# fanzyflani/pwnfps

Hardware: AMD Instinct MI355X
Metric: Mpixels/s at 3840x2160 (level.txt scene, trace + blur), frames resident on the device; mean steps/ray alongside; d2h_inclusive = the rate with every frame delivered to the host (SURVEY 8d) (higher is better)
Workload: dtype f32; 1 GPU; pwnfps level.txt scene (14 game.lua spheres, spawn pose, sec_current=0), 3840x2160, POSTPROC_BLUR=1, one frame per step; level=pwnfps_level, width=3840, height=2160, blur_passes=1, parallelism=rows/1, 3 frames in flight on two compute streams, frames_repeated_with_whole_strips=0

## Files before the change

pwnfps_amd/csrc/level_host.c:

```c
#include <stdint.h>
#include <stdlib.h>
#include <string.h>
#include "level_host.h"

enum { DIR_XP = 0, DIR_ZP, DIR_XN, DIR_ZN };

static int is_open(int c)
{
	switch(c)
	{
		case ';': case '$': case '"': case '#': case '&':
		case '>': case '<': case '^': case ',':
			return 1;
	}
	return 0;
}

static int flat_cell(const uint8_t *cells, int x, int z)
{
	int i = z * 64 + x;
	return (i >= 0 && i < 4096) ? cells[i] : '.';
}

static const int dir_dx[4] = { 1, 0, -1, 0 };
static const int dir_dz[4] = { 0, 1, 0, -1 };

static int open_dir(const uint8_t *cells, int x, int z)
{
	for(int d = 0; d < 4; d++)
		if(is_open(flat_cell(cells, x + dir_dx[d], z + dir_dz[d])))
			return d;
	return DIR_XP;
}

static void endpoint(pwn_portal *pm, int x, int z)
{
	if(pm->x1 == -1) { pm->x1 = x; pm->z1 = z; }
	else if(pm->x2 == -1) { pm->x2 = x; pm->z2 = z; }
}

void pwn_level_clear(uint8_t *cells, pwn_portal *pmap, int32_t *spawn)
{
	memset(cells, '.', 4096);
	for(int i = 0; i < 26; i++)
	{
		pmap[i].x1 = pmap[i].z1 = pmap[i].x2 = pmap[i].z2 = -1;
		pmap[i].rot12 = 0;
		pmap[i].c1 = pmap[i].c2 = ';';
	}
	spawn[0] = spawn[1] = 0;
}

int pwn_parse_level(const char *text, int len, uint8_t *cells, pwn_portal *pmap, int32_t *spawn)
{
	if(text == NULL || len < 0) return -1;
	pwn_level_clear(cells, pmap, spawn);

	const unsigned char *p = (const unsigned char *)text, *end = p + len;
	int x = 0, z = 0;
	while(p < end && z < 64)
	{
		int c = *p++;
		if(c == '\r' || c == '\n')
		{
			if(x != 0) { x = 0; z++; }
			continue;
		}
		if(c == '*') { spawn[0] = x; spawn[1] = z; c = ';'; }
		if(c >= 'a' && c < 'z')
		{
			endpoint(&pmap[c - 'a'], x, z);
			c = c - 'a' + 'A' + 1;
		}
		if(c >= 'A' && c <= 'Z') endpoint(&pmap[c - 'A'], x, z);
		cells[z * 64 + x] = (uint8_t)c;
		if(++x == 64) { x = 0; z++; }
	}

	for(int i = 0; i < 26; i++)
	{
		pwn_portal *pm = &pmap[i];
		if(pm->x2 == -1) continue;
		int d1 = open_dir(cells, pm->x1, pm->z1);
		int d2 = open_dir(cells, pm->x2, pm->z2);
		pm->rot12 = (d2 - d1 + 2) & 3;
		pm->c1 = flat_cell(cells, pm->x1 + dir_dx[d1], pm->z1 + dir_dz[d1]);
		pm->c2 = flat_cell(cells, pm->x2 + dir_dx[d2], pm->z2 + dir_dz[d2]);
	}
	return 0;
}

static int trunc_to_int(float f)
{
	return (f >= -2147483648.0f && f < 2147483648.0f) ? (int)f : INT32_MIN;
}

int pwn_bin_spheres(const pwn_sphere *s, int n, int32_t *off, int32_t *idx, int idx_cap)
{
	int32_t *fill = calloc(4096, sizeof(int32_t));
	if(fill == NULL) return -2;
	memset(off, 0, 4097 * sizeof(int32_t));
	for(int pass = 0; pass < 2; pass++)
	{
		for(int i = 0; i < n; i++)
		{
			int x1 = trunc_to_int(s[i].x - s[i].r), z1 = trunc_to_int(s[i].z - s[i].r);
			int x2 = trunc_to_int(s[i].x + s[i].r), z2 = trunc_to_int(s[i].z + s[i].r);
			if(x1 < 0) x1 = 0;
			if(z1 < 0) z1 = 0;
			if(x2 > 63) x2 = 63;
			if(z2 > 63) z2 = 63;
			for(int z = z1; z <= z2; z++)
			for(int x = x1; x <= x2; x++)
			{
				int c = z * 64 + x;
				if(pass == 0) off[c + 1]++;
				else idx[off[c] + fill[c]++] = i;
			}
		}
		if(pass == 0)
		{
			for(int c = 0; c < 4096; c++) off[c + 1] += off[c];
			if(idx == NULL) { free(fill); return off[4096]; }
			if(off[4096] > idx_cap) { free(fill); return -1; }
		}
	}
	free(fill);
	return off[4096];
}
```

pwnfps_amd/csrc/level_host.h:

```cpp
#ifndef PWN_LEVEL_HOST_H
#define PWN_LEVEL_HOST_H
#include <stdint.h>
#include "pwnhip.h"
#ifdef __cplusplus
extern "C" {
#endif
void pwn_level_clear(uint8_t *cells, pwn_portal *pmap, int32_t *spawn);
int pwn_parse_level(const char *text, int len, uint8_t *cells, pwn_portal *pmap, int32_t *spawn);
int pwn_bin_spheres(const pwn_sphere *s, int n, int32_t *off, int32_t *idx, int idx_cap);
#ifdef __cplusplus
}
#endif
#endif
```

pwnfps_amd/csrc/pwn_api.cpp:

```cpp
#include <hip/hip_runtime.h>
#include <stdint.h>
#include <stdio.h>
#include <stdlib.h>
#include <string.h>
#include <time.h>
#include <new>
#include <vector>
#include <xmmintrin.h>

#include "pwnhip.h"
#include "pwn_internal.h"
#include "level_host.h"
#include "approx_tables.inc"

extern "C" const char *pwn_strerror(int code)
{
	switch(code)
	{
		case PWN_OK: return "ok";
		case PWN_EINVAL: return "invalid argument";
		case PWN_ENODEV: return "no usable HIP device";
		case PWN_ENOMEM: return "out of memory";
		case PWN_EIO: return "level file could not be read";
		case PWN_EHIP: return "HIP runtime error";
// ... 241 lines not shown

extern "C" int pwn_set_option(pwn_ctx *c, int option, int value)
{
	if(GRP_HEAD(c)) return pwn_group_set_option(c, option, value);
	if(c == NULL) return PWN_EINVAL;
	switch(option)
	{
		case PWN_OPT_BLUR_PASSES:
			if(value < 0 || value > 16) return PWN_EINVAL;
			if(c->tiled != NULL) return PWN_EBUSY;
			for(int i = 0; i < c->nslots; i++) if(c->slot[i].in_flight) return PWN_EBUSY;
			c->blur_passes = value; return PWN_OK;
		case PWN_OPT_COUNTERS: c->counters_on = value ? 1 : 0; return PWN_OK;
		case PWN_OPT_SCHEDULER:
			if(value < 0 || value > PWN_SCHED_REFILL) return PWN_EINVAL;
			if(value != c->scheduler) c->blob_dirty = true;
			c->scheduler = value; return PWN_OK;
		case PWN_OPT_WAVE_LOG: c->wave_log_on = value ? 1 : 0; return PWN_OK;
		case PWN_OPT_FRAME_TIMING: if(value < 0) return PWN_EINVAL; c->frame_timing = value; return PWN_OK;
		case PWN_OPT_REFILL_LIMIT: if(value < 1 || value > 64000) return PWN_EINVAL; c->refill_limit = value; return PWN_OK;
		case PWN_OPT_UNIT_ORDER: if(value != 0 && value != 1) return PWN_EINVAL; c->unit_order = value; for(int i = 0; i < 4; i++) c->order[i].perm_valid = false; return PWN_OK;
		case PWN_OPT_TILED_CHOREO:
			if(value != PWN_TILED_CHOREO_INSTREAM && value != PWN_TILED_CHOREO_SPLIT) return PWN_EINVAL;
			if(c->tiled != NULL) return PWN_EBUSY;
			c->tiled_choreo = value; return PWN_OK;
		case PWN_OPT_TILED_COMMS:
			if(value != PWN_TILED_COMMS_ONE && value != PWN_TILED_COMMS_PER_STREAM) return PWN_EINVAL;
			if(c->tiled != NULL) return PWN_EBUSY;
			c->tiled_comms = value; return PWN_OK;
		case PWN_OPT_TILED_STREAMS:
			if(value != 2 && value != 3) return PWN_EINVAL;
			if(c->tiled != NULL) return PWN_EBUSY;
			c->tiled_streams = value; return PWN_OK;
		case PWN_OPT_TRACE_ROOM: if(value < -1 || value > 4096) return PWN_EINVAL; memset(&c->room, 0, sizeof(c->room)); c->room.mode = value; return PWN_OK;
		case PWN_OPT_CALL_STRIPS:
			if(value < -1 || value == 1 || value > PWN_CALL_STRIPS_MAX) return PWN_EINVAL;
			c->call_strips = value; c->strip_backoff = 0; c->strip_reach = 0; return PWN_OK;
		case PWN_OPT_FRAME_OVERLAP:
			for(int i = 0; i < c->nslots; i++) if(c->slot[i].in_flight) return PWN_EBUSY;
			c->frame_overlap = value ? 1 : 0; return PWN_OK;
	}
	return PWN_EINVAL;
}


static void expand_tables(uint16_t *rcp, uint16_t *rsq)
{
	for(int i = 0; i < 2048; i++)
	{
		rcp[i] = (uint16_t)(pwn_host_rcp_tab[i] ^ 0x1000u);
		rsq[i] = (uint16_t)(pwn_host_rsqrt_tab[i ^ 0x400] ^ 0x1000u);
	}
}

static int pack_blob(pwn_ctx *c)
{
	uint32_t nsph = (uint32_t)c->spheres.size();
	uint32_t nbin = 0;
	for(int i = 0; i < 4096; i++)
	{
		uint32_t cnt = (uint32_t)(c->bin_off[i + 1] - c->bin_off[i]);
		if(cnt) nbin += cnt + 1u;
	}
	if(nbin > 32767u || nsph * 32u >= PWN_LIST_END) return PWN_ETOOBIG;
	uint32_t total = (pwn_t_total(nbin, nsph) + 15u) & ~15u;
	if(total > PWN_BLOB_MAX) return PWN_ETOOBIG;
	uint32_t nrec = (uint32_t)c->bin_off[4096];
	bool inl = false;
	{
		const uint32_t total_inl = (pwn_t_total_inl(nrec, nsph) + 15u) & ~15u;
		const uint32_t extra = pwn_trace_lds_extra();
		const uint32_t fit_idx = 155648u / ((total + extra + 2047u) & ~2047u), fit_inl = 155648u / ((total_inl + extra + 2047u) & ~2047u);
		inl = c->scheduler == PWN_SCHED_UNITS && nrec > 0u && total_inl <= PWN_BLOB_MAX && fit_inl >= (fit_idx < 5u ? fit_idx : 5u);
		if(c->dbg_sphere_lists == 1) inl = false;
		if(c->dbg_sphere_lists == 2) inl = c->scheduler == PWN_SCHED_UNITS && nrec > 0u && total_inl <= PWN_BLOB_MAX;
		if(inl) total = total_inl;
	}
	c->blob.assign(total, 0);
	uint8_t *b = c->blob.data();
	uint32_t *ci = (uint32_t *)(b + PWN_T_CELLINFO);
	uint16_t *bi = (uint16_t *)(b + PWN_T_BINIDX);
	if(!c->cell_base_ok)
	{
		uint32_t *cb = c->cell_base;
		memset(cb, 0, sizeof(c->cell_base));
		for(int z = 0; z < 64; z++)
		for(int x = 0; x < 64; x++)
			cb[z * PWN_GRID_PITCH + x] = (uint32_t)c->cells[z * 64 + x] | pwn_cell_class(c->cells[z * 64 + x]);
		for(int z = 0; z < 64; z++) cb[z * PWN_GRID_PITCH + 64] = cb[z * PWN_GRID_PITCH];
		for(int x = 0; x <= 64; x++) cb[64 * PWN_GRID_PITCH + x] = cb[x];
		c->cell_base_ok = true;
	}
	memcpy(ci, c->cell_base, sizeof(c->cell_base));
	uint32_t at = 0;
	for(int i = 0; i < 4096 && !inl; i++)
	{
		int32_t k0 = c->bin_off[i], k1 = c->bin_off[i + 1];
		if(k1 > k0)
		{
			ci[(i >> 6) * PWN_GRID_PITCH + (i & 63)] |= PWN_C_SPH | (at << 16);
			for(int32_t k = k0; k < k1; k++) bi[at++] = (uint16_t)(c->bin_idx[k] * 32);
			bi[at++] = (uint16_t)PWN_LIST_END;
		}
	}
	if(inl)
	{
		float *rec = (float *)(b + PWN_T_BINIDX);
		uint16_t *which = (uint16_t *)(b + pwn_t_recsph_offset(nrec));
		for(int i = 0; i < 4096; i++)
		{
			const int32_t k0 = c->bin_off[i], k1 = c->bin_off[i + 1];
			if(k1 <= k0) continue;
			ci[(i >> 6) * PWN_GRID_PITCH + (i & 63)] |= PWN_C_SPH | ((uint32_t)k0 << 16);
			for(int32_t k = k0; k < k1; k++)
			{
				const pwn_sphere &q = c->spheres[(size_t)c->bin_idx[k]];
				float r2 = q.r * q.r;
				if(r2 < 1.17549435e-38f) r2 = 0.0f;
				rec[4 * k + 0] = q.x; rec[4 * k + 1] = q.y; rec[4 * k + 2] = q.z;
				uint32_t wbits;
				memcpy(&wbits, &r2, 4);
				if(k == k1 - 1) wbits |= 0x80000000u;
				memcpy(&rec[4 * k + 3], &wbits, 4);
				which[k] = (uint16_t)(c->bin_idx[k] * 32);
			}
		}
	}
	memcpy(b + PWN_T_RCP, c->tabs, 4096);
	memcpy(b + PWN_T_RSQ, c->tabs + 2048, 4096);
	pwn_fill_faces((float *)(b + PWN_T_FACES));
	uint32_t *pm = (uint32_t *)(b + PWN_T_PMAP);
	for(int i = 0; i < 26; i++)
	{
		const pwn_portal &p = c->pmap[i];
		pm[2 * i] = (uint32_t)(p.x1 & 0xff) | ((uint32_t)(p.z1 & 0xff) << 8) | ((uint32_t)(p.x2 & 0xff) << 16) | ((uint32_t)(p.z2 & 0xff) << 24);
		pm[2 * i + 1] = (uint32_t)(p.rot12 & 0xff) | ((uint32_t)(p.c1 & 0xff) << 8) | ((uint32_t)(p.c2 & 0xff) << 16);
	}
	c->off_sph = inl ? pwn_t_sph_offset_inl(nrec) : pwn_t_sph_offset(nbin);
	c->off_recsph = inl ? pwn_t_recsph_offset(nrec) : 0u;
	{
		float *sp = (float *)(b + c->off_sph);
		for(uint32_t i = 0; i < nsph; i++, sp += 8)
		{
			const pwn_sphere &q = c->spheres[i];
			float r2 = q.r * q.r;
			if(r2 < 1.17549435e-38f) r2 = 0.0f;
			sp[0] = q.x; sp[1] = q.y; sp[2] = q.z; sp[3] = r2;
			sp[4] = q.refl; sp[5] = q.cb; sp[6] = q.cg; sp[7] = q.cr;
		}
	}

	const int nb = (c->blob_cur + 1) % PWN_NBLOB;
	const uint32_t from = c->blob_has_static[nb] ? PWN_T_CELLINFO : 0u;
	const unsigned st = c->stage_next++ % PWN_NSTAGE;
	if(c->stage_used[st]) HIPCHK(c, hipEventSynchronize(c->ev_stage[st]));
	memcpy(c->h_stage[st], b + from, total - from);
	if(c->tables_in_use[nb]) HIPCHK(c, hipStreamWaitEvent(c->up_stream, c->tables_wait[nb], 0));
	HIPCHK(c, pwn_launch_upload(c->h_stage[st], c->d_blob[nb] + from, total - from, c->up_stream));
	HIPCHK(c, hipEventRecord(c->ev_stage[st], c->up_stream));
	HIPCHK(c, hipEventRecord(c->ev_upload[nb], c->up_stream));
	c->stage_used[st] = true;
	c->upload_pending[nb] = true;
	c->blob_has_static[nb] = true;
	c->blob_cur = nb;
	c->blob_dirty = false;
	return PWN_OK;
}

static int valid_portals(const pwn_portal *pm)
{
	for(int i = 0; i < 26; i++)
	{
		const int32_t v[4] = { pm[i].x1, pm[i].z1, pm[i].x2, pm[i].z2 };
		for(int k = 0; k < 4; k++) if(v[k] < -1 || v[k] > 63) return 0;
	}
	return 1;
}

extern "C" int pwn_upload_level(pwn_ctx *c, const uint8_t data[4096], const pwn_portal pmap[26])
{
	if(GRP_HEAD(c)) return (data == NULL || pmap == NULL) ? PWN_EINVAL : pwn_group_upload_level(c, data, pmap);
	if(c == NULL || data == NULL || pmap == NULL || !valid_portals(pmap)) return PWN_EINVAL;
	(void)hipSetDevice(c->device);
	memcpy(c->cells, data, 4096);
	memcpy(c->pmap, pmap, sizeof(c->pmap));
	c->have_level = true;
	c->cell_base_ok = false;
	c->blob_dirty = true;
	return pack_blob(c);
}

extern "C" int pwn_level_load_mem(pwn_ctx *c, const char *text, int len)
{
	if(GRP_HEAD(c)) return (text == NULL || len < 0) ? PWN_EINVAL : pwn_group_level_mem(c, text, len);
	if(c == NULL || text == NULL || len < 0) return PWN_EINVAL;
	(void)hipSetDevice(c->device);
	if(pwn_parse_level(text, len, c->cells, c->pmap, c->spawn) != 0) return PWN_EINVAL;
	c->have_level = true;
	c->cell_base_ok = false;
	c->blob_dirty = true;
	return pack_blob(c);
}

extern "C" int pwn_level_load(pwn_ctx *c, const char *path)
{
	if(c == NULL || path == NULL) return PWN_EINVAL;
	FILE *fp = fopen(path, "rb");
	if(fp == NULL) { snprintf(c->err, sizeof(c->err), "cannot open %s", path); return PWN_EIO; }
	std::vector<char> buf(1 << 20);
	size_t n = fread(buf.data(), 1, buf.size(), fp);
	fclose(fp);
	return pwn_level_load_mem(c, buf.data(), (int)n);
}

extern "C" int pwn_get_level(pwn_ctx *c, uint8_t data[4096], pwn_portal pmap[26], int32_t spawn[2])
{
	if(GRP_HEAD(c)) return pwn_get_level(GRP_M0(c), data, pmap, spawn);
	if(c == NULL) return PWN_EINVAL;
	if(data) memcpy(data, c->cells, 4096);
	if(pmap) memcpy(pmap, c->pmap, sizeof(c->pmap));
	if(spawn) { spawn[0] = c->spawn[0]; spawn[1] = c->spawn[1]; }
	return PWN_OK;
}

enum { OBJ_INVAL = 0, OBJ_FREE = 1, OBJ_SPHERE = 2 };

static int upload_live(pwn_ctx *c, const pwn_sphere *s, int n);

extern "C" int pwn_upload_spheres(pwn_ctx *c, const pwn_sphere *s, int n)
{
	if(GRP_HEAD(c)) return (n < 0 || n > PWN_OBJ_MAX || (n > 0 && s == NULL)) ? PWN_EINVAL : pwn_group_upload_spheres(c, s, n);
	if(c == NULL || n < 0 || n > PWN_OBJ_MAX || (n > 0 && s == NULL)) return PWN_EINVAL;
	int rc = upload_live(c, s, n);
	if(rc == PWN_OK)
	{
		c->objs.assign(s, s + n);
		c->obj_typ.assign((size_t)n, OBJ_SPHERE);
	}
	return rc;
}

extern "C" int pwn_obj_new(pwn_ctx *c)
{
	if(GRP_HEAD(c)) { const int r = pwn_obj_new(GRP_M0(c)); if(r < 0) snprintf(c->err, sizeof(c->err), "%s", GRP_M0(c)->err); return r; }
	if(c == NULL) return PWN_EINVAL;
	for(size_t i = 0; i < c->obj_typ.size(); i++)
		if(c->obj_typ[i] == OBJ_FREE) { c->obj_typ[i] = OBJ_INVAL; return (int)i; }
	if(c->obj_typ.size() >= (size_t)PWN_OBJ_MAX)
	{
		snprintf(c->err, sizeof(c->err), "obj_new: all %d object slots are taken", PWN_OBJ_MAX);
		return PWN_ENOMEM;
	}
	c->objs.push_back(pwn_sphere());
	c->obj_typ.push_back(OBJ_INVAL);
	return (int)c->obj_typ.size() - 1;
}

static bool obj_ok(pwn_ctx *c, int obj, const char *who)
{
	if(c == NULL) return false;
	if(obj >= 0 && (size_t)obj < c->obj_typ.size()) return true;
	snprintf(c->err, sizeof(c->err), "%s: %d is not an object", who, obj);
	return false;
}

// ... 1230 lines not shown
```

pwnfps_amd/csrc/pwn_internal.h:

```cpp
#pragma once
#include <hip/hip_runtime.h>
#include <stdint.h>
#include <stdio.h>
#include <vector>
#include <atomic>

#include "pwnhip.h"
#include "tables.h"

struct pwn_views_launch
{
	const pwn_view_rec *d_recs;
	int n;
	bool has_w;
	unsigned long long plane;
};

struct pwn_rays_launch
{
	const float *d_rays;
	const uint32_t *d_seeds;
	uint32_t n;
	bool has_w;
};
// ... 20 lines not shown
	int views;
};

extern "C" hipError_t pwn_launch_trace(const pwn_trace_params *P, int grid, size_t lds_bytes, bool count, hipStream_t stream);
extern "C" hipError_t pwn_launch_trace_refill(const pwn_trace_params *P, int grid, size_t lds_bytes, bool count, hipStream_t stream);
extern "C" unsigned pwn_trace_refill_lds_extra(bool has_w);
extern "C" int pwn_trace_refill_blocks_per_cu(size_t lds_bytes, bool count, bool has_w);
extern "C" int pwn_trace_blocks_per_cu(size_t lds_bytes, bool count, bool has_w);
extern "C" int pwn_trace_tile_h(void);
extern "C" int pwn_trace_tile_w(void);
extern "C" unsigned pwn_trace_lds_extra(void);
extern "C" hipError_t pwn_launch_blur(const pwn_blur_params *P, hipStream_t stream);
extern "C" hipError_t pwn_launch_order(const uint16_t *cost, uint32_t units, uint32_t cap, uint32_t *perm, hipStream_t stream);
extern "C" hipError_t pwn_launch_upscale(const uint32_t *src, uint32_t *dst, int w, int h, int scale, int pitch, hipStream_t stream);
extern "C" hipError_t pwn_launch_upload(const void *h_pinned_src, void *d_dst, size_t bytes, hipStream_t stream);
extern "C" hipError_t pwn_launch_words(const uint32_t *d_all, const uint32_t *d_own, uint32_t *h_pinned_dst, int world, hipStream_t stream);
extern "C" hipError_t pwn_launch_probe(int op, const uint32_t *in, uint32_t *out, int n, const uint16_t *tabs, hipStream_t stream);

#define PWN_BLOB_MAX (72u * 1024u)
#ifndef PWN_NBLOB
#define PWN_NBLOB 4
#endif
#define PWN_NCOUNTERS 48
#define PWN_TILED_STREAMS_DEFAULT 2
#define PWN_TICKET_SETS 6u
#define PWN_NSTAGE 4
#define PWN_CALL_STRIPS_MAX 32
#define PWN_HOST_REGS_MAX 16

struct pwn_slot
{
	uint32_t *d_out; float *d_z; uint32_t *d_surface;
	uint32_t *h_sbuf; float *h_zbuf; uint32_t *h_surface;
	hipEvent_t ev_k[4];
	hipEvent_t ev_done;
	bool in_flight, timed, beside;
	float sec;
	uint64_t seq;
};

struct pwn_room_ctl
{
	int mode;
	int arm, best;
	int skip, hold;
	double sum[2]; int cnt[2];
	double t_prev, t_hold;
	unsigned long long looks, switches;
};
int pwn_room_for_launch(struct pwn_ctx *c);
void pwn_room_frame_done(struct pwn_ctx *c);

struct pwn_tiled;
struct pwn_group;

#define PWN_HUB_RING 64
struct pwn_hub_post { void *dst; size_t bytes; hipEvent_t ev_free; int device; };
struct pwn_hub_box
{
	std::atomic<unsigned long long> posted, copied, consumed;
	pwn_hub_post post[PWN_HUB_RING];
	hipEvent_t done[PWN_HUB_RING];
};
struct pwn_hub
{
	int world;
	std::atomic<int> failed;
	std::atomic<unsigned> bar_count, bar_gen;
	struct pwn_ctx *member[PWN_TILED_MAX_WORLD];
	pwn_hub_box *boxes;
};
int pwn_hub_meet(pwn_hub *h, int wait_ms);

struct pwn_ctx
{
	int device, w, h;
	int num_cus;
	int blur_passes, counters_on, scheduler, refill_limit;
	bool have_level;

	uint8_t cells[4096];
	uint32_t cell_base[65 * 65];
	bool cell_base_ok;
	pwn_portal pmap[26];
	int32_t spawn[2];
	std::vector<pwn_sphere> spheres;
	std::vector<int32_t> bin_off, bin_idx;
	std::vector<pwn_sphere> objs;
	std::vector<uint8_t> obj_typ;

	std::vector<uint8_t> blob;
	uint8_t *d_blob[PWN_NBLOB]; int blob_cur;
	bool blob_has_static[PWN_NBLOB];
	hipEvent_t ev_tables[PWN_NBLOB]; bool tables_in_use[PWN_NBLOB];
	hipEvent_t tables_wait[PWN_NBLOB];
	hipEvent_t ev_upload[PWN_NBLOB]; bool upload_pending[PWN_NBLOB];
	uint8_t *h_stage[PWN_NSTAGE]; hipEvent_t ev_stage[PWN_NSTAGE]; bool stage_used[PWN_NSTAGE]; unsigned stage_next;
	hipStream_t up_stream;
	uint16_t tabs[4096];
	uint32_t off_sph;
	uint32_t off_recsph; int dbg_sphere_lists;
	bool blob_dirty;
	size_t occ_lds[8]; int occ_blocks[8];

	uint32_t *d_pre, *d_out;
	float *d_z;
	uint2 *d_skip;
	unsigned long long *d_counters;
	unsigned long long *d_wave_log; int wave_log_on; size_t wave_log_cap;
	struct unit_order_state
	{
		hipStream_t key; bool used; unsigned long long stamp;
		uint16_t *d_cost; uint32_t *d_perm; size_t cost_cap, perm_cap;
		uint32_t units, qcap; int y0, y1;
		bool cost_fresh;
		uint32_t perm_units; int perm_y0, perm_y1; bool perm_valid;
	} order[4];
	unsigned long long order_stamp;
	int tiled_choreo;
	int tiled_streams;
	int tiled_comms;
	int unit_order;
	unsigned long long order_used, order_sorts;
	bool dbg_force_hasw; int dbg_blocks_per_cu;
	int dbg_blur_th, dbg_blur_tw, dbg_blur_batch;
	int grid_reserve;
	uint32_t *d_vpre, *d_vout; float *d_vz; int views_cap;
	pwn_view_rec *h_vrec, *d_vrec; int vrec_cap;
	unsigned char *h_rays, *d_rays; size_t rays_cap;
	uint32_t *d_tickets; unsigned ticket_set;
	uint32_t *d_scratch; size_t scratch_cap;

	hipStream_t stream;
	hipStream_t stream2;
	uint32_t *d_pre2;
	pwn_room_ctl room;
	int frame_overlap;
	hipEvent_t last_frame_done; hipStream_t last_frame_stream;
	hipStream_t copy_stream;
	hipEvent_t ev[4];
	int call_strips;
	hipStream_t copy_stream2;
	int strip_copy_streams;
	int strip_calib_n; double strip_calib_ms[16];
	hipEvent_t strip_ev[2 * PWN_CALL_STRIPS_MAX]; int strip_ev_n;
	uint32_t *d_strip_miss, *h_strip_miss;
	int strips_last;
	int strip_reach;
	int strip_backoff;
	unsigned long long strip_calls, strip_redone;
	struct host_reg { void *base; size_t bytes; } host_regs[PWN_HOST_REGS_MAX]; int host_regs_n;
	pwn_stats stats;

	int nslots, frame_flags, frame_scale, frame_pitch, frame_timing;
	pwn_slot slot[PWN_MAX_SLOTS];
	uint64_t frame_seq;

	pwn_group *grp; bool grp_head;
	pwn_hub *hub;
	pwn_tiled *tiled;
	int tiled_init_ms, tiled_wait_ms;

	hipStream_t launch_stream[3]; hipEvent_t launch_event[3];
	unsigned long long launch_waits;
	int launch_rot;

// ... 42 lines not shown
```

pwnfps_amd/csrc/tables.h:

```cpp
#pragma once
#include <stdint.h>

#define PWN_GRID_PITCH 65u
#define PWN_T_RCP      0u
#define PWN_T_RSQ      4096u
#define PWN_T_FACES    8192u
#define PWN_T_EXP2     8448u
#define PWN_T_CELLINFO 8704u
#define PWN_T_PMAP     25616u
#define PWN_T_BINIDX   25824u

#define PWN_RCP_BASE   0x7e800000u
#define PWN_RSQ_BASE   0x5f000000u

#define PWN_C_ROOM   0x0100u
#define PWN_C_ROOM2  0x0200u
#define PWN_C_FOG    0x0400u
#define PWN_C_DQ     0x0800u
#define PWN_C_RAMP   0x1000u
#define PWN_C_RAMPX  0x2000u
#define PWN_C_RAMPM  0x4000u
#define PWN_C_PORTAL 0x8000u
#define PWN_C_SPH    0x80000000u
#define PWN_LIST_END 0xffffu

static inline uint32_t pwn_t_sph_offset(uint32_t nbin)
{
	return PWN_T_BINIDX + ((nbin * 2u + 15u) & ~15u);
}
static inline uint32_t pwn_t_total(uint32_t nbin, uint32_t nsph)
{
	return pwn_t_sph_offset(nbin) + nsph * 32u;
}
static inline uint32_t pwn_t_recsph_offset(uint32_t nrec) { return PWN_T_BINIDX + nrec * 16u; }
static inline uint32_t pwn_t_sph_offset_inl(uint32_t nrec) { return pwn_t_recsph_offset(nrec) + ((nrec * 2u + 15u) & ~15u); }
static inline uint32_t pwn_t_total_inl(uint32_t nrec, uint32_t nsph) { return pwn_t_sph_offset_inl(nrec) + nsph * 32u; }

#define PWN_EXP2F_TAB_INIT { \
	0x3ff0000000000000, 0x3fefd9b0d3158574, 0x3fefb5586cf9890f, 0x3fef9301d0125b51, \
	0x3fef72b83c7d517b, 0x3fef54873168b9aa, 0x3fef387a6e756238, 0x3fef1e9df51fdee1, \
	0x3fef06fe0a31b715, 0x3feef1a7373aa9cb, 0x3feedea64c123422, 0x3feece086061892d, \
	0x3feebfdad5362a27, 0x3feeb42b569d4f82, 0x3feeab07dd485429, 0x3feea47eb03a5585, \
	0x3feea09e667f3bcd, 0x3fee9f75e8ec5f74, 0x3feea11473eb0187, 0x3feea589994cce13, \
	0x3feeace5422aa0db, 0x3feeb737b0cdc5e5, 0x3feec49182a3f090, 0x3feed503b23e255d, \
	0x3feee89f995ad3ad, 0x3feeff76f2fb5e47, 0x3fef199bdd85529c, 0x3fef3720dcef9069, \
	0x3fef5818dcfba487, 0x3fef7c97337b9b5f, 0x3fefa4afa2a490da, 0x3fefd0765b6e4540 }

static inline void pwn_fill_faces(float *f)
{
	static const float col[4][4] = { { 30.0f, 30.0f, 0.0f, 0.0f }, { 1.0f, 1.0f, 1.0f, 0.0f }, { 0.8f, 0.8f, 1.0f, 0.0f }, { 5.0f, 0.0f, 5.0f, 0.0f } };
	for(int i = 0; i < 16; i++) f[i] = col[i >> 2][i & 3];
	uint32_t *u = (uint32_t *)(f + 16);
	const uint32_t S = 0x80000000u, P = 0x3a83126fu , N = 0xba83126fu, Z = 0x80000000u ;
	const uint32_t R25 = 0x3e800000u , R70 = 0x3f333333u ;
	const uint32_t t[6][8] = {
		{ S, 0, 0, R25,  N, Z, Z, 0 },
		{ 0, 0, S, R25,  Z, Z, N, 0 },
		{ S, 0, 0, R25,  P, Z, Z, S },
		{ 0, 0, S, R25,  Z, Z, P, S },
		{ 0, S, 0, R25,  Z, N, Z, 0 },
		{ 0, 0, 0, R70,  Z, N, Z, S },
	};
	for(int i = 0; i < 48; i++) u[i] = t[i >> 3][i & 7];
	static const uint64_t e2[32] = PWN_EXP2F_TAB_INIT;
	uint64_t *e = (uint64_t *)(f + (PWN_T_EXP2 - PWN_T_FACES) / 4u);
	for(int i = 0; i < 32; i++) e[i] = e2[i];
}

static inline uint32_t pwn_cell_class(uint32_t c)
{
	switch(c)
	{
		case ';': return PWN_C_ROOM;
		case '$': return PWN_C_ROOM | PWN_C_FOG;
		case '"': return PWN_C_ROOM | PWN_C_DQ;
		case '#': return PWN_C_ROOM | PWN_C_ROOM2;
		case '&': return PWN_C_ROOM | PWN_C_ROOM2 | PWN_C_FOG;
		case '>': return PWN_C_RAMP | PWN_C_RAMPX | PWN_C_RAMPM;
		case '<': return PWN_C_RAMP | PWN_C_RAMPX;
		case ',': return PWN_C_RAMP | PWN_C_RAMPM;
		case '^': return PWN_C_RAMP;
	}
	return (c >= 'A' && c <= 'Z') ? PWN_C_PORTAL : 0u;
}

struct pwn_trace_params
{
	float rayb[4], rdx[4], rdy[4], from[4];
	float sec_current;
	int w, h, y0, y1;
	int tiles_x, tiles_total;
	uint32_t ux_magic; int ux_shift;
	uint32_t blob_bytes, off_sph;
	uint32_t *sbuf;
	float *zbuf;
	const uint32_t *blob;
	unsigned long long *counters;
	unsigned long long *wave_log;
	int has_w;
	int scheduler;
	int refill_limit;
	uint32_t *tickets, *tickets_next;
	uint32_t *cost_word;
	uint16_t *unit_cost;
	const uint32_t *perm;
	uint32_t perm_cap;
	uint32_t *clear_word;
	uint32_t off_recsph;
	const struct pwn_view_rec *views;
	int nviews;
	uint32_t views_magic; int views_shift;
	unsigned long long plane;
	const float *rays;
	const uint32_t *ray_seeds;
	uint32_t nrays;
	int ray_w;
};

struct pwn_blur_params
{
	int w, h, y0, y1;
	int groups;
	const uint32_t *pre;
	const float *zbuf;
	uint32_t *out;
	const uint2 *skip;
	int avail_y0, avail_y1;
	uint32_t *miss;
	int tile_h, tile_w, batch;
	uint32_t *cost_acc, *cost_out;
	uint32_t cost_mul, cost_div;
	int views;
	unsigned long long plane;
};

enum { PWN_KM_FRAME = 0, PWN_KM_VIEWS = 1, PWN_KM_RAYS = 2 };

struct pwn_view_rec
{
	float rayb[4], rdx[4], rdy[4], from[4];
	float sec_current;
	float pad_[3];
};
#define PWN_VIEWS_REC_BYTES 80u

#ifndef PWN_QUEUES
#define PWN_QUEUES 64u
#endif
#define PWN_QUEUE_STRIDE 32u
```

pwnfps_amd/csrc/trace_common.h:

```cpp
#pragma once
#include <hip/hip_runtime.h>
#include "dev_math.h"
#include "tables.h"

#define EPS 0.0000000000001f
#define REFLECT_BLUR_F 0.03f
#define REFLECT_MAX 2
enum { FXP = 0, FZP, FXN, FZN, FYP, FYN };

#ifndef PWN_BLOCK
#define PWN_BLOCK 256
#endif
#define TILE_W 16
#define TILE_H 4

#ifndef PWN_MIN_WAVES
#define PWN_MIN_WAVES 3
#endif

#define PWN_LDS __attribute__((address_space(3)))
template<class T> __device__ __forceinline__ const PWN_LDS T *lds_at(uint32_t byte) { return (const PWN_LDS T *)(uintptr_t)byte; }
typedef float pwn_f4 __attribute__((ext_vector_type(4)));
struct Lds
{
	const PWN_LDS uint32_t *cellinfo;
	const PWN_LDS uint16_t *rcp, *rsq;
	const PWN_LDS uint32_t *pmap;
	const PWN_LDS uint16_t *binidx;
	const PWN_LDS uint16_t *recsph;
	const PWN_LDS float *sph;
	const PWN_LDS uint64_t *exp2;
	const PWN_LDS pwn_f4 *faces;
};
__device__ __forceinline__ Lds lds_tables(uint32_t off_sph, uint32_t off_recsph = 0u)
{
	Lds L;
	L.cellinfo = lds_at<uint32_t>(PWN_T_CELLINFO);
	L.rcp = lds_at<uint16_t>(PWN_T_RCP);
	L.rsq = lds_at<uint16_t>(PWN_T_RSQ);
	L.pmap = lds_at<uint32_t>(PWN_T_PMAP);
	L.binidx = lds_at<uint16_t>(PWN_T_BINIDX);
	L.faces = lds_at<pwn_f4>(PWN_T_FACES);
	L.exp2 = lds_at<uint64_t>(PWN_T_EXP2);
	L.sph = lds_at<float>(off_sph);
	L.recsph = lds_at<uint16_t>(off_recsph);
	return L;
}

__device__ __forceinline__ uint32_t cellword_at(const Lds &L, int cx, int cz)
{
	uint32_t ux = min((uint32_t)cx, 64u), uz = min((uint32_t)cz, 64u);
	return L.cellinfo[uz * PWN_GRID_PITCH + ux];
}

typedef unsigned short pwn_us2 __attribute__((ext_vector_type(2)));
typedef short pwn_s2 __attribute__((ext_vector_type(2)));
__device__ __forceinline__ uint32_t cxz_pack(int cx, int cz) { return ((uint32_t)cx & 0xffffu) | ((uint32_t)cz << 16); }
__device__ __forceinline__ uint32_t cxz_pack_start(int cx, int cz)
{
	return cxz_pack(max(min(cx, 16383), -16384), max(min(cz, 16383), -16384));
}
__device__ __forceinline__ int cxz_x(uint32_t c) { return (int)(int16_t)(uint16_t)(c & 0xffffu); }
__device__ __forceinline__ int cxz_z(uint32_t c) { return (int)c >> 16; }
__device__ __forceinline__ uint32_t cxz_add(uint32_t c, uint32_t step)
{
	return __builtin_bit_cast(uint32_t, (pwn_s2)(__builtin_bit_cast(pwn_s2, c) + __builtin_bit_cast(pwn_s2, step)));
}
__device__ __forceinline__ uint32_t cellword_pk(const Lds &L, uint32_t cxz)
{
	const pwn_us2 lim = { 64, 64 }, pitch = { 4, (unsigned short)(PWN_GRID_PITCH * 4u) };
	const pwn_us2 c = __builtin_elementwise_min(__builtin_bit_cast(pwn_us2, cxz), lim);
	const uint32_t byte = __builtin_amdgcn_udot2(c, pitch, 0u, false);
	return *(const PWN_LDS uint32_t *)((const PWN_LDS unsigned char *)L.cellinfo + byte);
}

template<bool HAS_W> struct Vec { float x, y, z, w; };

template<bool W> __device__ __forceinline__ float dot3(const Vec<W> &a, const Vec<W> &b)
{
	if constexpr(W) return (a.x * b.x + a.z * b.z) + (a.y * b.y + a.w * b.w);
	else return (a.x * b.x + a.z * b.z) + a.y * b.y;
}
template<bool W> __device__ __forceinline__ Vec<W> vscale(float s, const Vec<W> &a)
{
	Vec<W> r; r.x = s * a.x; r.y = s * a.y; r.z = s * a.z;
	if constexpr(W) r.w = s * a.w; else r.w = 0.0f;
	return r;
}
template<bool W> __device__ __forceinline__ Vec<W> vadd(const Vec<W> &a, const Vec<W> &b)
{
	Vec<W> r; r.x = a.x + b.x; r.y = a.y + b.y; r.z = a.z + b.z;
	if constexpr(W) r.w = a.w + b.w; else r.w = 0.0f;
	return r;
}
template<bool W> __device__ __forceinline__ Vec<W> vsub(const Vec<W> &a, const Vec<W> &b)
{
	Vec<W> r; r.x = a.x - b.x; r.y = a.y - b.y; r.z = a.z - b.z;
	if constexpr(W) r.w = a.w - b.w; else r.w = 0.0f;
	return r;
}
template<bool W> __device__ __forceinline__ Vec<W> vnormalise(const PWN_LDS uint16_t *rsq, const Vec<W> &a)
{
	return vscale<W>(tab_rsqrt(rsq, dot3<W>(a, a)), a);
}

__device__ __forceinline__ float dpp_row_shr1(float v)
{
	return __int_as_float(__builtin_amdgcn_update_dpp(0, __float_as_int(v), 0x111 , 0xf, 0xf, true));
}

enum { EV_NONE = 0, EV_WALL, EV_SPHERE, EV_EXHAUSTED };
enum { BASE_CEIL = 0, BASE_FLOOR, BASE_WALL, BASE_MAGENTA, BASE_ROOM_Y };

enum { RG_SEG = 0, RG_SETUP_SLOW, RG_EXHAUSTED, RG_WALL, RG_SPHERE, RG_FLOOR, RG_SPHREFL, RG_JITTER, RG_COMP1, RG_COMP1_FOG,
	RG_COMP2, RG_COMP2_FOG, RG_HELP, RG_UNIT, RG_SPHTEST, RG_SPHUPD, RG_ELSE,
	RG_UNIT_HALF, RG_HC_R2, RG_HC_OUT, RG_PORTAL_WALL, RG_PORTAL_GO, RG_PORTAL_ODD, RG_PORTAL_ROT2, RG_N };
struct Counters { uint32_t rays, steps, portals, tests, exhausted, wsteps, wp[8], apasses, apass_lanes, rg[RG_N]; };
#define WAVE_PATH(k) do { if(COUNT && (__ffsll((long long)__ballot(1)) - 1) == (int)(threadIdx.x & 63)) cnt.wp[k]++; } while(0)
#define RG(k) do { if(COUNT && (__ffsll((long long)__ballot(1)) - 1) == (int)(threadIdx.x & 63)) cnt.rg[k]++; } while(0)
```

pwnfps_amd/csrc/trace_walk.inc:

```
#define AUX_HIT() (cdist > aux_dist)
if(COUNT)
{
	cnt.steps++;
	if((__ffsll((long long)__ballot(1)) - 1) == (int)(threadIdx.x & 63)) cnt.wsteps++;
}

#ifdef PWN_PLAIN_STATS
if(COUNT)
{
	const bool sp1 = ((int)cw < 0) || !(cw & PWN_C_ROOM);
	const bool sp2 = sp1 || (cw & (PWN_C_ROOM2 | PWN_C_DQ)) != 0u;
	const bool low = (__ffsll((long long)__ballot(1)) - 1) == (int)(threadIdx.x & 63);
	if(__ballot(sp1) == 0ull && low) cnt.apasses++;
	if(__ballot(sp2) == 0ull && low) cnt.apass_lanes++;
}
#endif

if((int)cw < 0)
{
	WAVE_PATH(0);
	if constexpr(INL)
	{
		const PWN_LDS pwn_f4 *rp = (const PWN_LDS pwn_f4 *)L.binidx + ((cw >> 16) & 0x7fffu);
		pwn_f4 nx = *rp;
// ... 3 lines not shown
			const pwn_f4 s0 = nx;
			const uint32_t wb = __float_as_uint(s0.w);
			nx = rp[1];
#define PWN_ST_RAD2 __uint_as_float(wb & 0x7fffffffu)
#define PWN_ST_WHICH ((uint32_t)(uintptr_t)rp)
#include "trace_sphere.inc"
#undef PWN_ST_RAD2
#undef PWN_ST_WHICH
			if((int)wb < 0) break;
			rp++;
		}
	}
	else
	{
		const PWN_LDS uint16_t *lp = L.binidx + ((cw >> 16) & 0x7fffu);
		for(uint32_t si = *lp; si != PWN_LIST_END; si = *++lp)
		{
			RG(RG_SPHTEST);
			const pwn_f4 s0 = *(const PWN_LDS pwn_f4 *)((const PWN_LDS unsigned char *)L.sph + si);
#define PWN_ST_RAD2 s0.w
#define PWN_ST_WHICH si
#include "trace_sphere.inc"
#undef PWN_ST_RAD2
#undef PWN_ST_WHICH
		}
	}
}

if(cw & PWN_C_ROOM)
{
	WAVE_PATH(1);
	const bool room2 = (cw & PWN_C_ROOM2) != 0u;
	uint32_t m2;
	asm("v_bfe_i32 %0, %1, 9, 1" : "=v"(m2) : "v"(cw));
	static_assert(PWN_C_ROOM2 == (1u << 9), "v_bfe_i32 above reads bit 9");
	const float up2 = __uint_as_float(iay_up_bits & m2);
	wy += up2;
	const float cdist0 = cdist;
	const bool xlt = wx < wz;
	const float txz = xlt ? wx : wz;
	const bool ymin = wy < txz;
	const float t = ymin ? wy : txz;
	cdist += t;
	pos = vadd<HAS_W>(vscale<HAS_W>(t, ray), pos);
	const bool hit = AUX_HIT();
	if(cw & PWN_C_FOG)
	{
		WAVE_PATH(2);
		float fn = (fog - cdist0) + cdist;
		if(hit) fn = aux_dist > cdist0 ? (fog + aux_dist) - cdist0 : fog;
		fog = fn;
	}
	ldir = xlt ? ldx : ldz;
	ev = hit ? EV_SPHERE : (ymin ? EV_WALL : 0);
	wy = (wy - txz) - up2;
	wz = xlt ? wz - txz : iaz;
	wx = xlt ? iax : wx - txz;
	cxz = cxz_add(cxz, xlt ? sx : sz);
	const uint32_t ncw = cellword_pk(L, cxz);
	static_assert(PWN_C_DQ == (PWN_C_ROOM2 << 2), "the shift below lines DQ up with ROOM2");
	const uint32_t height_changes = (((cw >> 2) & ncw) | (cw & ~ncw)) & PWN_C_ROOM2;
	if(height_changes != 0u && !(hit || ymin))
	{
		WAVE_PATH(3);
		if(!room2)
		{
			if(ncw & PWN_C_ROOM2)
			{
				pos.y += 1.0f;
				wy -= iay_dn;
			}
		}
		else
		{
			RG(RG_HC_R2);
			if(ncw & PWN_C_DQ)
			{
				pos.y -= 1.0f;
				wy += iay_dn;
			}
			if(pos.y < 0.0f || pos.y > 1.0f)
			{
				RG(RG_HC_OUT);
				int xcell = (int)(ncw & 0xffu);
				if(ncw & PWN_C_PORTAL)
				{
					const int cx = cxz_x(cxz), cz = cxz_z(cxz);
					uint32_t p0 = L.pmap[2 * (xcell - 'A')], p1 = L.pmap[2 * (xcell - 'A') + 1];
					int x1 = (int)(int8_t)(p0 & 0xff), z1 = (int)(int8_t)((p0 >> 8) & 0xff);
					int x2 = (int)(int8_t)((p0 >> 16) & 0xff), z2 = (int)(int8_t)(p0 >> 24);
					if(x1 == cx && z1 == cz) xcell = (int)((p1 >> 16) & 0xff);
					else if(x2 == cx && z2 == cz) xcell = (int)((p1 >> 8) & 0xff);
				}
				if(!(xcell == '#' || xcell == '&'))
				{
					if(xcell == '"')
					{
						pos.y += 1.0f;
						wy -= iay_dn;
					}
					ev = EV_WALL; base = BASE_WALL;
				}
			}
		}
	}
	cw = ncw;
}
else
{
	RG(RG_ELSE);
	const uint32_t cw_in = cw;
	if(cw_in & PWN_C_RAMP)
	{
		WAVE_PATH(4);
		int cx = cxz_x(cxz), cz = cxz_z(cxz);
		const int gx = cxz_x(sx), gz = cxz_z(sz);
		const float ramp = 0.5f;
		const bool alongx = (cw & PWN_C_RAMPX) != 0u;
		const bool minus = (cw & PWN_C_RAMPM) != 0u;
		float tilt = alongx ? ray.x : ray.z;
		if(minus) ray.y -= ramp * tilt; else ray.y += ramp * tilt;
		wy = pos.y;
		if(ray.y >= 0.0f) wy = 1.0f - wy;
		wy *= 1.0f / (ray.y < 0.0f ? -ray.y : ray.y);
		if(AUX_HIT()) ev = EV_SPHERE;
		else
		{
			const bool ymin = (wy < wx) && (wy < wz);
			const bool xlt = wx < wz;
			const float t = ymin ? wy : (xlt ? wx : wz);
			cdist += t;
			pos = vadd<HAS_W>(vscale<HAS_W>(t, ray), pos);
			if(ymin)
			{
				ldir = (ray.y < 0.0f ? FYN : FYP);
				ev = EV_WALL; base = (ray.y >= 0.0f ? BASE_CEIL : BASE_FLOOR);
			}
			else
			{
				if(xlt)
				{
					ldir = (ray.x < 0.0f ? FXN : FXP);
					wy -= wx; wz -= wx; wx = iax; cx += gx;
				}
				else
				{
					ldir = (ray.z < 0.0f ? FZN : FZP);
					wx -= wz; wy -= wz; wz = iaz; cz += gz;
				}
				tilt = alongx ? ray.x : ray.z;
				if(minus) ray.y += ramp * tilt; else ray.y -= ramp * tilt;
				wy = pos.y;
				if(ray.y >= 0.0f) wy = 1.0f - wy;
				wy *= iay;
				cxz = cxz_pack(cx, cz);
				cw = cellword_pk(L, cxz);
			}
		}
	}
	if((cw_in & (PWN_C_RAMP | PWN_C_PORTAL)) == PWN_C_PORTAL)
	{
		WAVE_PATH(5);
		int cx = cxz_x(cxz), cz = cxz_z(cxz);
		int gx = cxz_x(sx), gz = cxz_z(sz);
		const int pi = (int)(cw & 0xffu) - 'A';
		uint32_t p0 = L.pmap[2 * pi], p1 = L.pmap[2 * pi + 1];
		int x1 = (int)(int8_t)(p0 & 0xff), z1 = (int)(int8_t)((p0 >> 8) & 0xff);
		int x2 = (int)(int8_t)((p0 >> 16) & 0xff), z2 = (int)(int8_t)(p0 >> 24);
		int rot12 = (int)(p1 & 0xff);
		const bool at1 = (x1 == cx && z1 == cz), at2 = (x2 == cx && z2 == cz);
		if(x2 == -1 || !(at1 || at2))
		{
			RG(RG_PORTAL_WALL);
			if(AUX_HIT()) ev = EV_SPHERE;
			else { ev = EV_WALL; base = (x2 == -1 ? BASE_WALL : BASE_MAGENTA); }
		}
		else
		{
			RG(RG_PORTAL_GO);
			int rot;
			if(at1)
			{
				cx = x2; cz = z2;
				pos.x += (float)(x2 - x1);
				pos.z += (float)(z2 - z1);
				rot = (-rot12) & 3;
			}
			else
			{
				cx = x1; cz = z1;
				pos.x -= (float)(x2 - x1);
				pos.z -= (float)(z2 - z1);
				rot = rot12 & 3;
			}
			if(COUNT) cnt.portals++;

			const float trx = pos.x, trz = pos.z, trvx = ray.x, trvz = ray.z;
			const int tgx = gx, tgz = gz;
			const float fcx = (float)cx, fcz = (float)cz;
			ldir = (ldir - rot) & 3;
			if(rot & 1)
			{
				RG(RG_PORTAL_ODD);
				float t = wx; wx = wz; wz = t;
				t = iax; iax = iaz; iaz = t;
				if(rot == 1)
				{
					pos.x = (trz + fcx) - fcz;
					pos.z = (1.0f - trx) + (fcx + fcz);
					ray.x = trvz; ray.z = -trvx;
					gx = tgz; gz = -tgx;
				}
				else
				{
					pos.x = (1.0f - trz) + (fcx + fcz);
					pos.z = (fcz + trx) - fcx;
					ray.x = -trvz; ray.z = trvx;
					gx = -tgz; gz = tgx;
				}
			}
			else if(rot == 2)
			{
				RG(RG_PORTAL_ROT2);
				pos.x = (fcx + 0.5f) * 2.0f - trx;
				pos.z = (fcz + 0.5f) * 2.0f - trz;
				ray.x = -trvx; ray.z = -trvz;
				gx = -tgx; gz = -tgz;
			}
			ldx = (gx < 0 ? FXN : FXP); ldz = (gz < 0 ? FZN : FZP);
			if(ldir == FZP) { cz++; pos.z += 1.0f; }
			else if(ldir == FXN) { cx--; pos.x -= 1.0f; }
			else if(ldir == FZN) { cz--; pos.z -= 1.0f; }
			else { cx++; pos.x += 1.0f; }
			cxz = cxz_pack(cx, cz);
			sx = (uint32_t)gx & 0xffffu; sz = (uint32_t)gz << 16;
			cw = cellword_pk(L, cxz);
		}
	}
	if((cw_in & (PWN_C_RAMP | PWN_C_PORTAL)) == 0u)
	{
		WAVE_PATH(6);
		if(AUX_HIT()) ev = EV_SPHERE;
		else { ev = EV_WALL; base = (ldir == FYP ? BASE_CEIL : BASE_WALL); }
	}
	if(ev == 0 && AUX_HIT()) ev = EV_SPHERE;
}
#undef AUX_HIT
```

Measured before the change: 26120 Mpixels/s.

## Bake portal endpoint state and look-through class into cell words

Precomputes per-cell portal state (wall, magenta, or an endpoint record index), the rotation, and the look-through class on the host. These are packed into the cell word, along with a small table of half-precision endpoint offsets. The trace kernel's portal and half-cell-out paths then replace the pmap lookup, endpoint coordinate compares and byte unpacking with bit tests and one LDS load. This reuses the ramp bits for the rotation and adds host-side validation of the outside-border portal cells.

```diff
diff --git a/pwnfps_amd/csrc/cell_bake.h b/pwnfps_amd/csrc/cell_bake.h
--- /dev/null
+++ b/pwnfps_amd/csrc/cell_bake.h
@@ -0,0 +1,16 @@
+#ifndef PWN_CELL_BAKE_H
+#define PWN_CELL_BAKE_H
+#include <stdint.h>
+
+#define PWN_C_LT2        0x01u
+#define PWN_C_LTDQ       0x02u
+#define PWN_C_PST_MASK   0xfcu
+#define PWN_C_PST_SHIFT  2u
+#define PWN_PST_WALL     0u
+#define PWN_PST_MAGENTA  1u
+#define PWN_PST_REC0     2u
+#define PWN_EP_MAX       52u
+
+#define PWN_C_PROT_SHIFT 13u
+
+#endif
diff --git a/pwnfps_amd/csrc/level_host.c b/pwnfps_amd/csrc/level_host.c
--- a/pwnfps_amd/csrc/level_host.c
+++ b/pwnfps_amd/csrc/level_host.c
@@ -88,6 +88,81 @@
 		pm->c2 = flat_cell(cells, pm->x2 + dir_dx[d2], pm->z2 + dir_dz[d2]);
 	}
 	return 0;
+}
+
+static uint32_t look_class(int c)
+{
+	if(c == '#' || c == '&') return PWN_C_LT2;
+	if(c == '"') return PWN_C_LTDQ;
+	return 0;
+}
+
+static int outside_cell_differs(const uint8_t *cells, const pwn_portal *pmap, int cx, int cz)
+{
+	const int c = cells[(cz < 0 ? 0 : cz) * 64 + (cx < 0 ? 0 : cx)];
+	if(c < 'A' || c > 'Z') return 0;
+	const pwn_portal *pm = &pmap[c - 'A'];
+	const int at1 = (pm->x1 == cx && pm->z1 == cz), at2 = (pm->x2 == cx && pm->z2 == cz);
+	if(at1) { if(look_class(pm->c2 & 0xff) != 0u) return 1; }
+	else if(at2) { if(look_class(pm->c1 & 0xff) != 0u) return 1; }
+	return pm->x2 != -1 && (at1 || at2);
+}
+
+int pwn_check_portals(const uint8_t *cells, const pwn_portal *pmap)
+{
+	for(int i = 0; i < 26; i++)
+	{
+		const int32_t v[4] = { pmap[i].x1, pmap[i].z1, pmap[i].x2, pmap[i].z2 };
+		for(int k = 0; k < 4; k++) if(v[k] < -1 || v[k] > 63) return 0;
+	}
+	for(int t = -1; t < 64; t++)
+		if(outside_cell_differs(cells, pmap, -1, t) || outside_cell_differs(cells, pmap, t, -1)) return 0;
+	return 1;
+}
+
+static uint32_t half_of_int(int v, int neg)
+{
+	uint32_t m = (uint32_t)(v < 0 ? -v : v), sign = (v < 0 || neg) ? 0x8000u : 0u;
+	if(m == 0) return sign;
+	int e = 0;
+	while((m >> e) > 1u) e++;
+	return sign | ((uint32_t)(e + 15) << 10) | ((m - (1u << e)) << (10 - e));
+}
+
+int pwn_bake_cells(const uint8_t *cells, const pwn_portal *pmap, uint16_t *bits, uint32_t *recs)
+{
+	int nrec = 0;
+	memset(bits, 0, 65 * 65 * sizeof(uint16_t));
+	memset(recs, 0, PWN_EP_MAX * sizeof(uint32_t));
+	for(int z = 0; z < 64; z++)
+	for(int x = 0; x < 64; x++)
+	{
+		const int c = cells[z * 64 + x];
+		uint32_t inside = look_class(c), outside = inside;
+		if(c >= 'A' && c <= 'Z')
+		{
+			const pwn_portal *pm = &pmap[c - 'A'];
+			const int at1 = (pm->x1 == x && pm->z1 == z), at2 = (pm->x2 == x && pm->z2 == z);
+			if(at1) inside = look_class(pm->c2 & 0xff);
+			else if(at2) inside = look_class(pm->c1 & 0xff);
+			uint32_t st = pm->x2 == -1 ? PWN_PST_WALL : PWN_PST_MAGENTA;
+			outside |= st << PWN_C_PST_SHIFT;
+			if(pm->x2 != -1 && (at1 || at2))
+			{
+				const int dx = pm->x2 - pm->x1, dz = pm->z2 - pm->z1;
+				recs[nrec] = at1 ? half_of_int(dx, 0) | (half_of_int(dz, 0) << 16)
+				                 : half_of_int(-dx, dx == 0) | (half_of_int(-dz, dz == 0) << 16);
+				inside |= ((at1 ? 0u - (uint32_t)pm->rot12 : (uint32_t)pm->rot12) & 3u) << PWN_C_PROT_SHIFT;
+				st = PWN_PST_REC0 + (uint32_t)nrec++;
+			}
+			inside |= st << PWN_C_PST_SHIFT;
+		}
+		bits[z * 65 + x] = (uint16_t)inside;
+		if(x == 0) bits[z * 65 + 64] = (uint16_t)outside;
+		if(z == 0) bits[64 * 65 + x] = (uint16_t)outside;
+		if(x == 0 && z == 0) bits[64 * 65 + 64] = (uint16_t)outside;
+	}
+	return nrec;
 }
 
 static int trunc_to_int(float f)
diff --git a/pwnfps_amd/csrc/level_host.h b/pwnfps_amd/csrc/level_host.h
--- a/pwnfps_amd/csrc/level_host.h
+++ b/pwnfps_amd/csrc/level_host.h
@@ -2,11 +2,14 @@
 #define PWN_LEVEL_HOST_H
 #include <stdint.h>
 #include "pwnhip.h"
+#include "cell_bake.h"
 #ifdef __cplusplus
 extern "C" {
 #endif
 void pwn_level_clear(uint8_t *cells, pwn_portal *pmap, int32_t *spawn);
 int pwn_parse_level(const char *text, int len, uint8_t *cells, pwn_portal *pmap, int32_t *spawn);
+int pwn_check_portals(const uint8_t *cells, const pwn_portal *pmap);
+int pwn_bake_cells(const uint8_t *cells, const pwn_portal *pmap, uint16_t *bits, uint32_t *recs);
 int pwn_bin_spheres(const pwn_sphere *s, int n, int32_t *off, int32_t *idx, int idx_cap);
 #ifdef __cplusplus
 }
diff --git a/pwnfps_amd/csrc/pwn_api.cpp b/pwnfps_amd/csrc/pwn_api.cpp
--- a/pwnfps_amd/csrc/pwn_api.cpp
+++ b/pwnfps_amd/csrc/pwn_api.cpp
@@ -347,13 +347,11 @@
 	uint16_t *bi = (uint16_t *)(b + PWN_T_BINIDX);
 	if(!c->cell_base_ok)
 	{
-		uint32_t *cb = c->cell_base;
-		memset(cb, 0, sizeof(c->cell_base));
-		for(int z = 0; z < 64; z++)
-		for(int x = 0; x < 64; x++)
-			cb[z * PWN_GRID_PITCH + x] = (uint32_t)c->cells[z * 64 + x] | pwn_cell_class(c->cells[z * 64 + x]);
-		for(int z = 0; z < 64; z++) cb[z * PWN_GRID_PITCH + 64] = cb[z * PWN_GRID_PITCH];
-		for(int x = 0; x <= 64; x++) cb[64 * PWN_GRID_PITCH + x] = cb[x];
+		std::vector<uint16_t> bits(65 * 65);
+		pwn_bake_cells(c->cells, c->pmap, bits.data(), c->ep_recs);
+		for(int z = 0; z <= 64; z++)
+		for(int x = 0; x <= 64; x++)
+			c->cell_base[z * PWN_GRID_PITCH + x] = (uint32_t)bits[z * PWN_GRID_PITCH + x] | pwn_cell_class(c->cells[(z & 63) * 64 + (x & 63)]);
 		c->cell_base_ok = true;
 	}
 	memcpy(ci, c->cell_base, sizeof(c->cell_base));
@@ -394,13 +392,7 @@
 	memcpy(b + PWN_T_RCP, c->tabs, 4096);
 	memcpy(b + PWN_T_RSQ, c->tabs + 2048, 4096);
 	pwn_fill_faces((float *)(b + PWN_T_FACES));
-	uint32_t *pm = (uint32_t *)(b + PWN_T_PMAP);
-	for(int i = 0; i < 26; i++)
-	{
-		const pwn_portal &p = c->pmap[i];
-		pm[2 * i] = (uint32_t)(p.x1 & 0xff) | ((uint32_t)(p.z1 & 0xff) << 8) | ((uint32_t)(p.x2 & 0xff) << 16) | ((uint32_t)(p.z2 & 0xff) << 24);
-		pm[2 * i + 1] = (uint32_t)(p.rot12 & 0xff) | ((uint32_t)(p.c1 & 0xff) << 8) | ((uint32_t)(p.c2 & 0xff) << 16);
-	}
+	memcpy(b + PWN_T_EPREC, c->ep_recs, sizeof(c->ep_recs));
 	c->off_sph = inl ? pwn_t_sph_offset_inl(nrec) : pwn_t_sph_offset(nbin);
 	c->off_recsph = inl ? pwn_t_recsph_offset(nrec) : 0u;
 	{
@@ -432,20 +424,10 @@
 	return PWN_OK;
 }
 
-static int valid_portals(const pwn_portal *pm)
-{
-	for(int i = 0; i < 26; i++)
-	{
-		const int32_t v[4] = { pm[i].x1, pm[i].z1, pm[i].x2, pm[i].z2 };
-		for(int k = 0; k < 4; k++) if(v[k] < -1 || v[k] > 63) return 0;
-	}
-	return 1;
-}
-
 extern "C" int pwn_upload_level(pwn_ctx *c, const uint8_t data[4096], const pwn_portal pmap[26])
 {
 	if(GRP_HEAD(c)) return (data == NULL || pmap == NULL) ? PWN_EINVAL : pwn_group_upload_level(c, data, pmap);
-	if(c == NULL || data == NULL || pmap == NULL || !valid_portals(pmap)) return PWN_EINVAL;
+	if(c == NULL || data == NULL || pmap == NULL || !pwn_check_portals(data, pmap)) return PWN_EINVAL;
 	(void)hipSetDevice(c->device);
 	memcpy(c->cells, data, 4096);
 	memcpy(c->pmap, pmap, sizeof(c->pmap));
diff --git a/pwnfps_amd/csrc/pwn_internal.h b/pwnfps_amd/csrc/pwn_internal.h
--- a/pwnfps_amd/csrc/pwn_internal.h
+++ b/pwnfps_amd/csrc/pwn_internal.h
@@ -126,6 +126,7 @@
 	uint8_t cells[4096];
 	uint32_t cell_base[65 * 65];
 	bool cell_base_ok;
+	uint32_t ep_recs[PWN_EP_MAX];
 	pwn_portal pmap[26];
 	int32_t spawn[2];
 	std::vector<pwn_sphere> spheres;
diff --git a/pwnfps_amd/csrc/tables.h b/pwnfps_amd/csrc/tables.h
--- a/pwnfps_amd/csrc/tables.h
+++ b/pwnfps_amd/csrc/tables.h
@@ -1,5 +1,6 @@
 #pragma once
 #include <stdint.h>
+#include "cell_bake.h"
 
 #define PWN_GRID_PITCH 65u
 #define PWN_T_RCP      0u
@@ -7,7 +8,7 @@
 #define PWN_T_FACES    8192u
 #define PWN_T_EXP2     8448u
 #define PWN_T_CELLINFO 8704u
-#define PWN_T_PMAP     25616u
+#define PWN_T_EPREC    25616u
 #define PWN_T_BINIDX   25824u
 
 #define PWN_RCP_BASE   0x7e800000u
@@ -67,7 +68,7 @@
 	for(int i = 0; i < 32; i++) e[i] = e2[i];
 }
 
-static inline uint32_t pwn_cell_class(uint32_t c)
+static constexpr inline uint32_t pwn_cell_class(uint32_t c)
 {
 	switch(c)
 	{
diff --git a/pwnfps_amd/csrc/trace_common.h b/pwnfps_amd/csrc/trace_common.h
--- a/pwnfps_amd/csrc/trace_common.h
+++ b/pwnfps_amd/csrc/trace_common.h
@@ -25,7 +25,7 @@
 {
 	const PWN_LDS uint32_t *cellinfo;
 	const PWN_LDS uint16_t *rcp, *rsq;
-	const PWN_LDS uint32_t *pmap;
+	const PWN_LDS unsigned char *eprec;
 	const PWN_LDS uint16_t *binidx;
 	const PWN_LDS uint16_t *recsph;
 	const PWN_LDS float *sph;
@@ -38,7 +38,7 @@
 	L.cellinfo = lds_at<uint32_t>(PWN_T_CELLINFO);
 	L.rcp = lds_at<uint16_t>(PWN_T_RCP);
 	L.rsq = lds_at<uint16_t>(PWN_T_RSQ);
-	L.pmap = lds_at<uint32_t>(PWN_T_PMAP);
+	L.eprec = lds_at<unsigned char>(PWN_T_EPREC - PWN_PST_REC0 * 4u);
 	L.binidx = lds_at<uint16_t>(PWN_T_BINIDX);
 	L.faces = lds_at<pwn_f4>(PWN_T_FACES);
 	L.exp2 = lds_at<uint64_t>(PWN_T_EXP2);
@@ -72,6 +72,16 @@
 	const pwn_us2 c = __builtin_elementwise_min(__builtin_bit_cast(pwn_us2, cxz), lim);
 	const uint32_t byte = __builtin_amdgcn_udot2(c, pitch, 0u, false);
 	return *(const PWN_LDS uint32_t *)((const PWN_LDS unsigned char *)L.cellinfo + byte);
+}
+
+static_assert(PWN_C_PST_SHIFT == 2u && PWN_T_EPREC + PWN_EP_MAX * 4u <= PWN_T_BINIDX, "ep_rec takes the state field as a byte offset; 52 records fit");
+static_assert(PWN_C_RAMPX == (1u << PWN_C_PROT_SHIFT) && PWN_C_RAMPM == (2u << PWN_C_PROT_SHIFT), "the rotation takes the place of RAMPX | RAMPM");
+static_assert(pwn_cell_class('A') == PWN_C_PORTAL && pwn_cell_class('M') == PWN_C_PORTAL && pwn_cell_class('Z') == PWN_C_PORTAL, "a letter's cell has no ramp bit");
+static_assert((PWN_C_PST_MASK | PWN_C_LT2 | PWN_C_LTDQ) == 0xffu, "the baked byte lies below the class bits");
+typedef _Float16 pwn_h2 __attribute__((ext_vector_type(2)));
+__device__ __forceinline__ pwn_h2 ep_rec(const Lds &L, uint32_t pst_in_place)
+{
+	return __builtin_bit_cast(pwn_h2, *(const PWN_LDS uint32_t *)(L.eprec + pst_in_place));
 }
 
 template<bool HAS_W> struct Vec { float x, y, z, w; };
diff --git a/pwnfps_amd/csrc/trace_walk.inc b/pwnfps_amd/csrc/trace_walk.inc
--- a/pwnfps_amd/csrc/trace_walk.inc
+++ b/pwnfps_amd/csrc/trace_walk.inc
@@ -109,19 +109,9 @@
 			if(pos.y < 0.0f || pos.y > 1.0f)
 			{
 				RG(RG_HC_OUT);
-				int xcell = (int)(ncw & 0xffu);
-				if(ncw & PWN_C_PORTAL)
-				{
-					const int cx = cxz_x(cxz), cz = cxz_z(cxz);
-					uint32_t p0 = L.pmap[2 * (xcell - 'A')], p1 = L.pmap[2 * (xcell - 'A') + 1];
-					int x1 = (int)(int8_t)(p0 & 0xff), z1 = (int)(int8_t)((p0 >> 8) & 0xff);
-					int x2 = (int)(int8_t)((p0 >> 16) & 0xff), z2 = (int)(int8_t)(p0 >> 24);
-					if(x1 == cx && z1 == cz) xcell = (int)((p1 >> 16) & 0xff);
-					else if(x2 == cx && z2 == cz) xcell = (int)((p1 >> 8) & 0xff);
-				}
-				if(!(xcell == '#' || xcell == '&'))
-				{
-					if(xcell == '"')
+				if(!(ncw & PWN_C_LT2))
+				{
+					if(ncw & PWN_C_LTDQ)
 					{
 						pos.y += 1.0f;
 						wy -= iay_dn;
@@ -188,43 +178,29 @@
 	if((cw_in & (PWN_C_RAMP | PWN_C_PORTAL)) == PWN_C_PORTAL)
 	{
 		WAVE_PATH(5);
-		int cx = cxz_x(cxz), cz = cxz_z(cxz);
-		int gx = cxz_x(sx), gz = cxz_z(sz);
-		const int pi = (int)(cw & 0xffu) - 'A';
-		uint32_t p0 = L.pmap[2 * pi], p1 = L.pmap[2 * pi + 1];
-		int x1 = (int)(int8_t)(p0 & 0xff), z1 = (int)(int8_t)((p0 >> 8) & 0xff);
-		int x2 = (int)(int8_t)((p0 >> 16) & 0xff), z2 = (int)(int8_t)(p0 >> 24);
-		int rot12 = (int)(p1 & 0xff);
-		const bool at1 = (x1 == cx && z1 == cz), at2 = (x2 == cx && z2 == cz);
-		if(x2 == -1 || !(at1 || at2))
+		const uint32_t pst = cw_in & PWN_C_PST_MASK;
+		if(pst < (PWN_PST_REC0 << PWN_C_PST_SHIFT))
 		{
 			RG(RG_PORTAL_WALL);
+			static_assert(BASE_WALL + PWN_PST_WALL == BASE_WALL && BASE_WALL + PWN_PST_MAGENTA == BASE_MAGENTA, "the state is the wall class");
 			if(AUX_HIT()) ev = EV_SPHERE;
-			else { ev = EV_WALL; base = (x2 == -1 ? BASE_WALL : BASE_MAGENTA); }
+			else { ev = EV_WALL; base = BASE_WALL + (int)(pst >> PWN_C_PST_SHIFT); }
 		}
 		else
 		{
 			RG(RG_PORTAL_GO);
-			int rot;
-			if(at1)
-			{
-				cx = x2; cz = z2;
-				pos.x += (float)(x2 - x1);
-				pos.z += (float)(z2 - z1);
-				rot = (-rot12) & 3;
-			}
-			else
-			{
-				cx = x1; cz = z1;
-				pos.x -= (float)(x2 - x1);
-				pos.z -= (float)(z2 - z1);
-				rot = rot12 & 3;
-			}
+			const pwn_h2 er = ep_rec(L, pst);
+			const float edx = (float)er.x, edz = (float)er.y;
+			int gx = cxz_x(sx), gz = cxz_z(sz);
+			pos.x += edx;
+			pos.z += edz;
+			const int rot = (int)((cw_in >> PWN_C_PROT_SHIFT) & 3u);
 			if(COUNT) cnt.portals++;
 
 			const float trx = pos.x, trz = pos.z, trvx = ray.x, trvz = ray.z;
 			const int tgx = gx, tgz = gz;
-			const float fcx = (float)cx, fcz = (float)cz;
+			const float fcx = (float)cxz_x(cxz) + edx, fcz = (float)cxz_z(cxz) + edz;
+			int cx = (int)fcx, cz = (int)fcz;
 			ldir = (ldir - rot) & 3;
 			if(rot & 1)
 			{
```

Result: faster. 26850 Mpixels/s, median of 6 (+2.8%).
